# aynik/carta1

Hardware: AMD Instinct MI355X
Metric: atrac1_stereo_frames_per_s_encode (higher is better)
Workload: dtype f32+f64

## Files before the change

### carta1_amd/csrc/c1_k_analysis.hip

```cpp
#include "c1_device.h"

namespace {

struct alignas(16) LongLds {
  float d1[46];
  float d2[46];
  uint32_t late[4][64];
  uint32_t sfw[64];
  double win[32];
  alignas(16) float hbuf[296];
  alignas(4) uint8_t sfi[64];
  union alignas(16) {
    struct { alignas(16) double w1[698]; } q1;
    struct { alignas(16) double w2[454]; } q2;
    struct {
      union alignas(16) {
        struct { alignas(16) float in0[256]; alignas(16) float in1[256]; alignas(16) float in2[512]; } i;
        struct { alignas(16) float coef[512]; } c;
      } a;
      union alignas(16) { float band[512]; } zz;
    } m;
    struct { alignas(16) float skip_[896]; float2 z[320]; } zp;
  } u;
};

struct alignas(16) MixedLds {
  double d1[46];
  double d2[46];
  alignas(16) float band[512];
  alignas(16) float hbuf[296];
  alignas(4) uint8_t sfi[64];
  alignas(16) float ovl[96];
  union alignas(16) {
    struct { alignas(16) double w1[698]; } q1;
    struct { alignas(16) double w2[454]; } q2;
    struct {
      union alignas(16) {
        struct { alignas(16) float in[1120]; } g;
        struct { alignas(16) float coef[512]; } c;
      } a;
      union alignas(16) { float2 z[320]; } zz;
    } m;
  } u;
};

template <bool ALL_LONG>
__global__ __launch_bounds__(C1_WAVE, ALL_LONG ? 4 : 3) void k_analysis_fast(C1EncodeLaunch L) {
  using Lds = typename std::conditional<ALL_LONG, LongLds, MixedLds>::type;
  __shared__ Lds S;
  float *band_;
  if constexpr (ALL_LONG) band_ = S.u.m.zz.band; else band_ = S.band;
  const C1DevEncOpts *O = L.opts;
  const int lane0 = threadIdx.x;
  int lane = lane0;
  const bool listed = L.unit_list != nullptr;
  const int64_t n_items = listed ? (int64_t)*L.unit_count : (int64_t)gridDim.x;
  R4Geometry G4 = r4_geometry(lane0);
  const SfLong SFL = sf_long_geometry(lane0);
  if constexpr (ALL_LONG) {
#pragma unroll
    for (int j = 0; j < 4; j++) {
      S.late[j][lane0] = r4_late_word(G4, j);
      G4.cx[j] = G4.cy[j] = G4.post_tab[j] = 0;
    }
    S.sfw[lane0] = (uint32_t)SFL.src | ((uint32_t)SFL.b << 13) | (SFL.wide ? 1u << 19 : 0u) | (SFL.store ? 1u << 20 : 0u);
    if (lane0 < 32) S.win[lane0] = C1_TABLES(L.tables)->window[lane0];
  }
  const SfLong SFM = sf_geometry(lane0, O->modes[0], O->modes[1], O->modes[2]);
  const MixGeometry GM = mix_geometry(lane0, FrameModes{O->modes[0], O->modes[1], O->modes[2]});
  const TablesRsrc RT = tables_rsrc(L.tables);
  for (int64_t item = blockIdx.x; item < n_items; item += gridDim.x) {
  const int64_t listed_unit = listed ? (int64_t)L.unit_list[item] : 0;
  const int ch = listed ? (int)(listed_unit % L.channels) : (int)(blockIdx.x % L.channels);
  const int64_t f0 = listed ? listed_unit / L.channels : (int64_t)(blockIdx.x / L.channels) * L.run_frames;
  const int64_t run_frames = listed ? (L.list_runs ? (f0 / L.run_frames + 1) * L.run_frames - f0 : 1) : L.run_frames;
  const float *__restrict__ pcm = L.pcm[ch];
  lane = lane0;

  for (int i = lane; i < 46; i += 64) { S.d1[i] = 0.0; S.d2[i] = 0.0; }
  for (int i = lane; i < 296; i += 64) S.hbuf[i] = 0.0f;
  if (lane < 12) S.sfi[52 + lane] = 0;
  if constexpr (!ALL_LONG) {
    for (int i = lane; i < 96; i += 64) S.ovl[i] = 0.0f;
  }
  float ov0 = 0.0f, ov1 = 0.0f, ov2 = 0.0f;
  wave_fence();

  const int64_t f_end = (f0 + run_frames < L.frames) ? f0 + run_frames : L.frames;
  constexpr int kWarm = 1;
  int64_t f_first = f0 - kWarm;
  if (f_first < -(int64_t)L.halo_frames) f_first = -(int64_t)L.halo_frames;
  if (f_first > f0) f_first = f0;
  typedef float v4f __attribute__((ext_vector_type(4)));
  v4f pre_a, pre_b;
  auto deliver = [&]() {
    asm volatile("" : "+v"(pre_a), "+v"(pre_b));
  };
  {
    const v4f *p4 = reinterpret_cast<const v4f *>(pcm + f_first * 512);
    pre_a = p4[lane0]; pre_b = p4[64 + lane0];
    deliver();
  }
  for (int64_t f = f_first; f < f_end; ++f) {
    const bool emit = (f >= f0);
    TablesPtr T = tables_for_this_frame(L.tables);
    lane = lane_for_this_frame(lane0);

    {
      const v4f a = pre_a, b = pre_b;
      {
        const v4f *p4 = reinterpret_cast<const v4f *>(pcm + ((f + 1 < f_end) ? f + 1 : f) * 512);
        pre_a = p4[lane]; pre_b = p4[64 + lane];
      }
      double *w1 = S.u.q1.w1;
      if (lane < 46) w1[pidx<3>(lane)] = S.d1[lane];
      const int e0 = 46 + 4 * lane;
      *reinterpret_cast<double2 *>(&w1[pidx<3>(e0)]) = make_double2((double)a.x, (double)a.y);
      *reinterpret_cast<double2 *>(&w1[pidx<3>(e0 + 2)]) = make_double2((double)a.z, (double)a.w);
      *reinterpret_cast<double2 *>(&w1[pidx<3>(e0 + 256)]) = make_double2((double)b.x, (double)b.y);
      *reinterpret_cast<double2 *>(&w1[pidx<3>(e0 + 258)]) = make_double2((double)b.z, (double)b.w);
    }
    wave_fence();
    {
      double ev[4], od[4];
      if constexpr (ALL_LONG) __builtin_amdgcn_s_setprio(3);
      if (own_block()) qmf_analysis_core<4, 3>(S.u.q1.w1, lane, T, ev, od); else { for (int d = 0; d < 4; d++) { ev[d] = S.u.q1.w1[lane + d]; od[d] = 1.0; } }
      double *w2 = S.u.q2.w2;
      if (lane < 46) { w2[pidx<2>(lane)] = S.d2[lane]; S.d1[lane] = S.u.q1.w1[pidx<3>(512 + lane)]; }
      float lo[4];
#pragma unroll
      for (int d = 0; d < 4; d++) {
        lo[d] = f32(ev[d] + od[d]);
        S.hbuf[39 + 4 * lane + d] = f32(ev[d] - od[d]);
      }
      *reinterpret_cast<double2 *>(&w2[pidx<2>(46 + 4 * lane)]) = make_double2((double)lo[0], (double)lo[1]);
      *reinterpret_cast<double2 *>(&w2[pidx<2>(48 + 4 * lane)]) = make_double2((double)lo[2], (double)lo[3]);
    }
    wave_fence();
    R4Early EARLY;
    if constexpr (ALL_LONG) EARLY = r4_early(G4, RT);
    {
      double ev[2], od[2];
      if (own_block()) qmf_analysis_core<2, 2>(S.u.q2.w2, lane, T, ev, od); else { for (int d = 0; d < 2; d++) { ev[d] = S.u.q2.w2[lane + d]; od[d] = 1.0; } }
      if constexpr (ALL_LONG) __builtin_amdgcn_s_setprio(1);
      *reinterpret_cast<float2 *>(&band_[2 * lane]) = make_float2(f32(ev[0] + od[0]), f32(ev[1] + od[1]));
      *reinterpret_cast<float2 *>(&band_[128 + 2 * lane]) = make_float2(f32(ev[0] - od[0]), f32(ev[1] - od[1]));
      *reinterpret_cast<float4 *>(&band_[256 + 4 * lane]) = *reinterpret_cast<const float4 *>(&S.hbuf[4 * lane]);
      if (lane < 46) S.d2[lane] = S.u.q2.w2[pidx<2>(256 + lane)];
    }
    wave_fence();
    {
      float keep = 0.0f;
      if (lane < 39) keep = S.hbuf[256 + lane];
      wave_fence();
      if (lane < 39) S.hbuf[lane] = keep;
    }
    deliver();
    if (emit && L.bands) {
      float4 *dst = reinterpret_cast<float4 *>(L.bands + ((f * L.channels + ch) << 9));
      const float4 *src = reinterpret_cast<const float4 *>(band_);
      dst[lane] = src[lane];
      dst[64 + lane] = src[64 + lane];
    }

    if constexpr (ALL_LONG) {
      float *in0 = S.u.m.a.i.in0, *in1 = S.u.m.a.i.in1, *in2 = S.u.m.a.i.in2;
      float nov0 = 0.0f, nov1 = 0.0f, nov2 = 0.0f;
      if (lane < 32) {
        const double w_lo = S.win[lane], w_hi = S.win[31 - lane];
        const double x0 = band_[96 + lane], x1 = band_[128 + 96 + lane], x2 = band_[256 + 224 + lane];
        nov0 = f32(w_lo * x0); nov1 = f32(w_lo * x1); nov2 = f32(w_lo * x2);
        if (emit) {
          in0[48 + lane] = ov0; in1[48 + lane] = ov1; in2[112 + lane] = ov2;
          in0[80 + 96 + lane] = f32(x0 * w_hi);
          in1[80 + 96 + lane] = f32(x1 * w_hi);
          in2[144 + 224 + lane] = f32(x2 * w_hi);
        }
      }
      ov0 = nov0; ov1 = nov1; ov2 = nov2;
      if (!emit) { wave_fence(); continue; }
      {
        const float4 zero4 = make_float4(0.0f, 0.0f, 0.0f, 0.0f);
        if (lane < 48) {
          float *inb = lane < 24 ? in0 : in1;
          const int q = lane < 24 ? lane : lane - 24;
          *reinterpret_cast<float4 *>(&inb[q < 12 ? 4 * q : 208 + 4 * (q - 12)]) = zero4;
        }
        if (lane < 56) *reinterpret_cast<float4 *>(&in2[lane < 28 ? 4 * lane : 400 + 4 * (lane - 28)]) = zero4;
        if (lane < 48) {
          *reinterpret_cast<float2 *>(&in0[80 + 2 * lane]) = *reinterpret_cast<const float2 *>(&band_[2 * lane]);
          *reinterpret_cast<float2 *>(&in1[80 + 2 * lane]) = *reinterpret_cast<const float2 *>(&band_[128 + 2 * lane]);
        }
        if (lane < 56) *reinterpret_cast<float4 *>(&in2[144 + 4 * lane]) = *reinterpret_cast<const float4 *>(&band_[256 + 4 * lane]);
      }
      wave_fence();
      float *coef = S.u.m.a.c.coef;
      __builtin_amdgcn_s_setprio(0);
      mdct_long_r4(in0, S.u.zp.z, coef, G4, T, RT, EARLY, &S.late[0][0] + lane);
      __builtin_amdgcn_s_setprio(1);
      wave_fence();

      const int64_t unit = f * L.channels + ch;
      {
        const uint32_t sw = S.sfw[lane];
        const float4 *grp = reinterpret_cast<const float4 *>(coef + (sw & 0x1fcu));
        float mx = sf_scan_long_groups(grp[0], grp[1], grp[2]);
        const float other = __int_as_float(__builtin_amdgcn_update_dpp(0, __float_as_int(mx), 0xB1, 0xf, 0xf, false));
        mx = fmaxf(mx, ((sw >> 19) & 1u) ? other : 0.0f);
        const int sfi = scale_factor_index_fast(mx, T->sf_m1, T->sf_m2);
        if ((sw >> 20) & 1u) S.sfi[(sw >> 13) & 63u] = (uint8_t)sfi;
      }
      {
        float4 *dst = reinterpret_cast<float4 *>(L.coefs + (unit << 9));
        const float4 *src = reinterpret_cast<const float4 *>(coef);
        dst[lane] = src[lane];
        dst[64 + lane] = src[64 + lane];
      }
      wave_fence();
      if (lane < 16) reinterpret_cast<uint32_t *>(L.side + unit * kSideBytes)[lane] = reinterpret_cast<const uint32_t *>(S.sfi)[lane];
      if ((L.list_runs || L.list_zero_eps) && lane == 16) *reinterpret_cast<float4 *>(L.eps + unit * kEpsFloats) = make_float4(0.0f, 0.0f, 0.0f, 0.0f);
      wave_fence();
    } else {
      const FrameModes M{O->modes[0], O->modes[1], O->modes[2]};
      float *coef = S.u.m.a.c.coef;
      if (emit) {
        mix_stage(band_, S.ovl, S.u.m.a.g.in, M, lane, RT);
        wave_fence();
        mdct_mixed_r4(S.u.m.a.g.in, S.u.m.zz.z, coef, GM, M.m0 == 0 || M.m1 == 0 || M.m2 == 0, M.m2 == 0, T, RT);
      }
      for (int i = lane; i < 96; i += 64) {
        const int b = i >> 5, k = i & 31;
        const int Sb = b == 2 ? 256 : 128, off = b == 0 ? 0 : (b == 1 ? 128 : 256);
        S.ovl[i] = f32(T->window[k] * (double)band_[off + Sb - 32 + k]);
      }
      wave_fence();
      if (!emit) continue;

      const int64_t unit = f * L.channels + ch;
      {
        float4 *dst = reinterpret_cast<float4 *>(L.coefs + (unit << 9));
        const float4 *src = reinterpret_cast<const float4 *>(coef);
        dst[lane] = src[lane];
        dst[64 + lane] = src[64 + lane];
      }
      sf_long(coef, S.sfi, SFM, T);
      if (lane >= 60 && lane < 63) reinterpret_cast<uint32_t *>(S.sfi)[13 + (lane - 60)] = lane == 60 ? (uint32_t)((M.m0 & 3) | ((M.m1 & 3) << 2) | ((M.m2 & 3) << 4)) : 0u;
      wave_fence();
      if (lane < 16) reinterpret_cast<uint32_t *>(L.side + unit * kSideBytes)[lane] = reinterpret_cast<const uint32_t *>(S.sfi)[lane];
      if ((L.list_runs || L.list_zero_eps) && lane == 16) *reinterpret_cast<float4 *>(L.eps + unit * kEpsFloats) = make_float4(0.0f, 0.0f, 0.0f, 0.0f);
      wave_fence();
    }
  }
  wave_fence();
  }
}

}

void c1k_launch_analysis(const C1EncodeLaunch &L0, bool detect, hipStream_t stream) {
  static const int slots = c1k_wave_slots(k_analysis_fast<false>);
  C1EncodeLaunch L = L0;
  L.run_frames = c1k_pick_run(L.frames, L.channels, slots);
  const int64_t runs = (L.frames + L.run_frames - 1) / L.run_frames;
  const int64_t blocks = L.unit_list ? std::min<int64_t>(L.frames * L.channels, 256 * 12) : runs * L.channels;
  const dim3 grid((unsigned)blocks), block(C1_WAVE);
  (void)detect;
  hipLaunchKernelGGL((k_analysis_fast<false>), grid, block, 0, stream, L);
}
void c1k_launch_analysis_long(const C1EncodeLaunch &L0, hipStream_t stream) {
  static const int slots = c1k_wave_slots(k_analysis_fast<true>);
  C1EncodeLaunch L = L0;
  L.run_frames = c1k_pick_run(L.frames, L.channels, slots);
  const int64_t runs = (L.frames + L.run_frames - 1) / L.run_frames;
  const int64_t blocks = L.unit_list ? std::min<int64_t>(L.frames * L.channels, 256 * 16) : runs * L.channels;
  hipLaunchKernelGGL((k_analysis_fast<true>), dim3((unsigned)blocks), dim3(C1_WAVE), 0, stream, L);
}
static_assert(sizeof(LongLds) <= 10240, "all-long analysis: 16 waves per CU (4 per SIMD, 128 registers) need <= 10 KiB of LDS per wave");
```

Measured before the change: 197.6 million.

## Specialise all-long analysis kernel with contiguous LDS QMF windows and cross-item prefetch

```diff
diff --git a/carta1_amd/csrc/c1_k_analysis.hip b/carta1_amd/csrc/c1_k_analysis.hip
--- a/carta1_amd/csrc/c1_k_analysis.hip
+++ b/carta1_amd/csrc/c1_k_analysis.hip
@@ -1,17 +1,18 @@
 #include "c1_device.h"
 
+#include <cstddef>
+
 namespace {
 
 struct alignas(16) LongLds {
-  float d1[46];
-  float d2[46];
   uint32_t late[4][64];
   uint32_t sfw[64];
   double win[32];
-  alignas(16) float hbuf[296];
+  double d2[48];
   alignas(4) uint8_t sfi[64];
+  alignas(16) double h1[60];
   union alignas(16) {
-    struct { alignas(16) double w1[698]; } q1;
+    struct { alignas(16) double w1_body[638]; } q1;
     struct { alignas(16) double w2[454]; } q2;
     struct {
       union alignas(16) {
@@ -22,7 +23,13 @@
     } m;
     struct { alignas(16) float skip_[896]; float2 z[320]; } zp;
   } u;
+  float hi_tail[64];
 };
+constexpr int kLongW1 = offsetof(LongLds, h1), kLongUnion = offsetof(LongLds, u), kLongBand = kLongUnion + 4096;
+static_assert(kLongUnion - kLongW1 == 60 * 8, "w1's head ends where its body starts");
+static_assert(sizeof(LongLds::u) == 6144 && offsetof(LongLds, hi_tail) == kLongBand + 2048, "hi_tail continues band");
+static_assert(kLongW1 % 16 == 0 && kLongUnion % 16 == 0, "16-byte window reads");
+static_assert(sizeof(LongLds) <= 10240, "all-long analysis: 16 waves per CU (4 per SIMD, 128 registers) need <= 10 KiB of LDS per wave");
 
 struct alignas(16) MixedLds {
   double d1[46];
@@ -45,27 +52,15 @@
 };
 
 template <bool ALL_LONG>
-__global__ __launch_bounds__(C1_WAVE, ALL_LONG ? 4 : 3) void k_analysis_fast(C1EncodeLaunch L) {
-  using Lds = typename std::conditional<ALL_LONG, LongLds, MixedLds>::type;
-  __shared__ Lds S;
-  float *band_;
-  if constexpr (ALL_LONG) band_ = S.u.m.zz.band; else band_ = S.band;
+__global__ __launch_bounds__(C1_WAVE, 3) void k_analysis_fast(C1EncodeLaunch L) {
+  static_assert(!ALL_LONG, "the all-long kernel is the specialisation below");
+  __shared__ MixedLds S;
+  float *band_ = S.band;
   const C1DevEncOpts *O = L.opts;
   const int lane0 = threadIdx.x;
   int lane = lane0;
   const bool listed = L.unit_list != nullptr;
   const int64_t n_items = listed ? (int64_t)*L.unit_count : (int64_t)gridDim.x;
-  R4Geometry G4 = r4_geometry(lane0);
-  const SfLong SFL = sf_long_geometry(lane0);
-  if constexpr (ALL_LONG) {
-#pragma unroll
-    for (int j = 0; j < 4; j++) {
-      S.late[j][lane0] = r4_late_word(G4, j);
-      G4.cx[j] = G4.cy[j] = G4.post_tab[j] = 0;
-    }
-    S.sfw[lane0] = (uint32_t)SFL.src | ((uint32_t)SFL.b << 13) | (SFL.wide ? 1u << 19 : 0u) | (SFL.store ? 1u << 20 : 0u);
-    if (lane0 < 32) S.win[lane0] = C1_TABLES(L.tables)->window[lane0];
-  }
   const SfLong SFM = sf_geometry(lane0, O->modes[0], O->modes[1], O->modes[2]);
   const MixGeometry GM = mix_geometry(lane0, FrameModes{O->modes[0], O->modes[1], O->modes[2]});
   const TablesRsrc RT = tables_rsrc(L.tables);
@@ -80,10 +75,7 @@
   for (int i = lane; i < 46; i += 64) { S.d1[i] = 0.0; S.d2[i] = 0.0; }
   for (int i = lane; i < 296; i += 64) S.hbuf[i] = 0.0f;
   if (lane < 12) S.sfi[52 + lane] = 0;
-  if constexpr (!ALL_LONG) {
-    for (int i = lane; i < 96; i += 64) S.ovl[i] = 0.0f;
-  }
-  float ov0 = 0.0f, ov1 = 0.0f, ov2 = 0.0f;
+  for (int i = lane; i < 96; i += 64) S.ovl[i] = 0.0f;
   wave_fence();
 
   const int64_t f_end = (f0 + run_frames < L.frames) ? f0 + run_frames : L.frames;
@@ -123,7 +115,6 @@
     wave_fence();
     {
       double ev[4], od[4];
-      if constexpr (ALL_LONG) __builtin_amdgcn_s_setprio(3);
       if (own_block()) qmf_analysis_core<4, 3>(S.u.q1.w1, lane, T, ev, od); else { for (int d = 0; d < 4; d++) { ev[d] = S.u.q1.w1[lane + d]; od[d] = 1.0; } }
       double *w2 = S.u.q2.w2;
       if (lane < 46) { w2[pidx<2>(lane)] = S.d2[lane]; S.d1[lane] = S.u.q1.w1[pidx<3>(512 + lane)]; }
@@ -137,12 +128,9 @@
       *reinterpret_cast<double2 *>(&w2[pidx<2>(48 + 4 * lane)]) = make_double2((double)lo[2], (double)lo[3]);
     }
     wave_fence();
-    R4Early EARLY;
-    if constexpr (ALL_LONG) EARLY = r4_early(G4, RT);
     {
       double ev[2], od[2];
       if (own_block()) qmf_analysis_core<2, 2>(S.u.q2.w2, lane, T, ev, od); else { for (int d = 0; d < 2; d++) { ev[d] = S.u.q2.w2[lane + d]; od[d] = 1.0; } }
-      if constexpr (ALL_LONG) __builtin_amdgcn_s_setprio(1);
       *reinterpret_cast<float2 *>(&band_[2 * lane]) = make_float2(f32(ev[0] + od[0]), f32(ev[1] + od[1]));
       *reinterpret_cast<float2 *>(&band_[128 + 2 * lane]) = make_float2(f32(ev[0] - od[0]), f32(ev[1] - od[1]));
       *reinterpret_cast<float4 *>(&band_[256 + 4 * lane]) = *reinterpret_cast<const float4 *>(&S.hbuf[4 * lane]);
@@ -163,64 +151,7 @@
       dst[64 + lane] = src[64 + lane];
     }
 
-    if constexpr (ALL_LONG) {
-      float *in0 = S.u.m.a.i.in0, *in1 = S.u.m.a.i.in1, *in2 = S.u.m.a.i.in2;
-      float nov0 = 0.0f, nov1 = 0.0f, nov2 = 0.0f;
-      if (lane < 32) {
-        const double w_lo = S.win[lane], w_hi = S.win[31 - lane];
-        const double x0 = band_[96 + lane], x1 = band_[128 + 96 + lane], x2 = band_[256 + 224 + lane];
-        nov0 = f32(w_lo * x0); nov1 = f32(w_lo * x1); nov2 = f32(w_lo * x2);
-        if (emit) {
-          in0[48 + lane] = ov0; in1[48 + lane] = ov1; in2[112 + lane] = ov2;
-          in0[80 + 96 + lane] = f32(x0 * w_hi);
-          in1[80 + 96 + lane] = f32(x1 * w_hi);
-          in2[144 + 224 + lane] = f32(x2 * w_hi);
-        }
-      }
-      ov0 = nov0; ov1 = nov1; ov2 = nov2;
-      if (!emit) { wave_fence(); continue; }
-      {
-        const float4 zero4 = make_float4(0.0f, 0.0f, 0.0f, 0.0f);
-        if (lane < 48) {
-          float *inb = lane < 24 ? in0 : in1;
-          const int q = lane < 24 ? lane : lane - 24;
-          *reinterpret_cast<float4 *>(&inb[q < 12 ? 4 * q : 208 + 4 * (q - 12)]) = zero4;
-        }
-        if (lane < 56) *reinterpret_cast<float4 *>(&in2[lane < 28 ? 4 * lane : 400 + 4 * (lane - 28)]) = zero4;
-        if (lane < 48) {
-          *reinterpret_cast<float2 *>(&in0[80 + 2 * lane]) = *reinterpret_cast<const float2 *>(&band_[2 * lane]);
-          *reinterpret_cast<float2 *>(&in1[80 + 2 * lane]) = *reinterpret_cast<const float2 *>(&band_[128 + 2 * lane]);
-        }
-        if (lane < 56) *reinterpret_cast<float4 *>(&in2[144 + 4 * lane]) = *reinterpret_cast<const float4 *>(&band_[256 + 4 * lane]);
-      }
-      wave_fence();
-      float *coef = S.u.m.a.c.coef;
-      __builtin_amdgcn_s_setprio(0);
-      mdct_long_r4(in0, S.u.zp.z, coef, G4, T, RT, EARLY, &S.late[0][0] + lane);
-      __builtin_amdgcn_s_setprio(1);
-      wave_fence();
-
-      const int64_t unit = f * L.channels + ch;
-      {
-        const uint32_t sw = S.sfw[lane];
-        const float4 *grp = reinterpret_cast<const float4 *>(coef + (sw & 0x1fcu));
-        float mx = sf_scan_long_groups(grp[0], grp[1], grp[2]);
-        const float other = __int_as_float(__builtin_amdgcn_update_dpp(0, __float_as_int(mx), 0xB1, 0xf, 0xf, false));
-        mx = fmaxf(mx, ((sw >> 19) & 1u) ? other : 0.0f);
-        const int sfi = scale_factor_index_fast(mx, T->sf_m1, T->sf_m2);
-        if ((sw >> 20) & 1u) S.sfi[(sw >> 13) & 63u] = (uint8_t)sfi;
-      }
-      {
-        float4 *dst = reinterpret_cast<float4 *>(L.coefs + (unit << 9));
-        const float4 *src = reinterpret_cast<const float4 *>(coef);
-        dst[lane] = src[lane];
-        dst[64 + lane] = src[64 + lane];
-      }
-      wave_fence();
-      if (lane < 16) reinterpret_cast<uint32_t *>(L.side + unit * kSideBytes)[lane] = reinterpret_cast<const uint32_t *>(S.sfi)[lane];
-      if ((L.list_runs || L.list_zero_eps) && lane == 16) *reinterpret_cast<float4 *>(L.eps + unit * kEpsFloats) = make_float4(0.0f, 0.0f, 0.0f, 0.0f);
-      wave_fence();
-    } else {
+    {
       const FrameModes M{O->modes[0], O->modes[1], O->modes[2]};
       float *coef = S.u.m.a.c.coef;
       if (emit) {
@@ -252,6 +183,243 @@
     }
   }
   wave_fence();
+  }
+}
+
+template <int D, int S>
+__device__ __forceinline__ void qmf_core_long(const double *w, int lane, TablesPtr T, double (&even)[D], double (&odd)[D]) {
+  static_assert(2 * D == (1 << S), "the lane base is affine only then");
+  const double *base = w + (2 * D + 2) * lane;
+#pragma unroll
+  for (int d = 0; d < D; d++) even[d] = odd[d] = 0.0;
+#pragma unroll
+  for (int u = 22 + D; u >= 0; --u) {
+    constexpr int kTwo = 2;
+    const int q = kTwo + 2 * u;
+    const double2 x = *reinterpret_cast<const double2 *>(base + (q + 2 * (q >> S)));
+#pragma unroll
+    for (int d = 0; d < D; d++) {
+      const int j = d + 23 - u;
+      if (j >= 0 && j < 24) {
+        odd[d] = __builtin_fma(x.x, T->tap_e[23 - j], odd[d]);
+        even[d] = __builtin_fma(x.y, T->tap_e[j], even[d]);
+      }
+    }
+  }
+}
+
+struct LongItem {
+  int ch;
+  int64_t f0, f_first, f_end;
+};
+
+template <>
+__global__ __launch_bounds__(C1_WAVE, 4) void k_analysis_fast<true>(C1EncodeLaunch L) {
+  __shared__ LongLds S;
+  double *const w1 = reinterpret_cast<double *>(reinterpret_cast<char *>(&S) + kLongW1);
+  double *const w2 = S.u.q2.w2;
+  float *const band_ = reinterpret_cast<float *>(reinterpret_cast<char *>(&S) + kLongBand);
+  const int lane0 = threadIdx.x;
+  int lane = lane0;
+  const bool listed = L.unit_list != nullptr;
+  const int64_t n_items = listed ? (int64_t)*L.unit_count : (int64_t)gridDim.x;
+  if ((int64_t)blockIdx.x >= n_items) return;
+  R4Geometry G4 = r4_geometry(lane0);
+  const SfLong SFL = sf_long_geometry(lane0);
+#pragma unroll
+  for (int j = 0; j < 4; j++) {
+    S.late[j][lane0] = r4_late_word(G4, j);
+    G4.cx[j] = G4.cy[j] = G4.post_tab[j] = 0;
+  }
+  S.sfw[lane0] = (uint32_t)SFL.src | ((uint32_t)SFL.b << 13) | (SFL.wide ? 1u << 19 : 0u) | (SFL.store ? 1u << 20 : 0u);
+  if (lane0 < 32) S.win[lane0] = C1_TABLES(L.tables)->window[lane0];
+  if (lane0 < 12) S.sfi[52 + lane0] = 0;
+  const TablesRsrc RT = tables_rsrc(L.tables);
+
+  auto item_of = [&](uint32_t unit) -> LongItem {
+    LongItem I;
+    int64_t run;
+    if (listed) {
+      const uint32_t nch = (uint32_t)L.channels;
+      uint32_t fr;
+      if (nch == 2u) { I.ch = (int)(unit & 1u); fr = unit >> 1; }
+      else if (nch == 1u) { I.ch = 0; fr = unit; }
+      else { I.ch = (int)(unit % nch); fr = unit / nch; }
+      I.f0 = (int64_t)fr;
+      run = L.list_runs ? (int64_t)((uint32_t)L.run_frames - fr % (uint32_t)L.run_frames) : 1;
+    } else {
+      I.ch = (int)(blockIdx.x % L.channels);
+      I.f0 = (int64_t)(blockIdx.x / L.channels) * L.run_frames;
+      run = L.run_frames;
+    }
+    I.f_end = (I.f0 + run < L.frames) ? I.f0 + run : L.frames;
+    constexpr int kWarm = 1;
+    I.f_first = I.f0 - kWarm;
+    if (I.f_first < -(int64_t)L.halo_frames) I.f_first = -(int64_t)L.halo_frames;
+    if (I.f_first > I.f0) I.f_first = I.f0;
+    return I;
+  };
+  typedef const __attribute__((address_space(4))) uint32_t *ListPtr;
+  auto word_at = [&](int64_t i) -> uint32_t { return (listed && i < n_items) ? ((ListPtr)L.unit_list)[i] : 0u; };
+
+  typedef float v4f __attribute__((ext_vector_type(4)));
+  v4f pre_a, pre_b;
+  auto deliver = [&]() {
+    asm volatile("" : "+v"(pre_a), "+v"(pre_b));
+  };
+  int64_t item = blockIdx.x;
+  uint32_t word = word_at(item), word_next = word_at(item + gridDim.x);
+  {
+    const LongItem I = item_of(__builtin_amdgcn_readfirstlane(word));
+    const v4f *p4 = reinterpret_cast<const v4f *>(L.pcm[I.ch] + I.f_first * 512);
+    pre_a = p4[lane0]; pre_b = p4[64 + lane0];
+    deliver();
+  }
+  for (;;) {
+  const int64_t next_item = item + gridDim.x;
+  const bool more = next_item < n_items;
+  const uint32_t word_after = word_at(next_item + gridDim.x);
+  const LongItem I = item_of(__builtin_amdgcn_readfirstlane(word));
+  const int ch = I.ch;
+  const int64_t f0 = I.f0, f_first = I.f_first, f_end = I.f_end;
+  const float *__restrict__ pcm = L.pcm[ch];
+  const float *after = pcm + (f_end - 1) * 512;
+  if (more) {
+    const LongItem N = item_of(__builtin_amdgcn_readfirstlane(word_next));
+    after = L.pcm[N.ch] + N.f_first * 512;
+  }
+  lane = lane0;
+
+  if (f_first == f0) {
+    if (lane < 60) w1[lane] = 0.0;
+    if (lane < 48) S.d2[lane] = 0.0;
+    band_[512 + lane] = 0.0f;
+  }
+  float ov0 = 0.0f, ov1 = 0.0f, ov2 = 0.0f;
+  wave_fence();
+
+  for (int64_t f = f_first; f < f_end; ++f) {
+    const bool emit = (f >= f0);
+    TablesPtr T = tables_for_this_frame(L.tables);
+    lane = lane_for_this_frame(lane0);
+
+    {
+      const v4f a = pre_a, b = pre_b;
+      {
+        const v4f *p4 = reinterpret_cast<const v4f *>((f + 1 < f_end) ? pcm + (f + 1) * 512 : after);
+        pre_a = p4[lane]; pre_b = p4[64 + lane];
+      }
+      double *at = w1 + (60 + 5 * lane - (lane & 1));
+      *reinterpret_cast<double2 *>(at) = make_double2((double)a.x, (double)a.y);
+      *reinterpret_cast<double2 *>(at + 2) = make_double2((double)a.z, (double)a.w);
+      *reinterpret_cast<double2 *>(at + 320) = make_double2((double)b.x, (double)b.y);
+      *reinterpret_cast<double2 *>(at + 322) = make_double2((double)b.z, (double)b.w);
+    }
+    wave_fence();
+    {
+      double ev[4], od[4];
+      __builtin_amdgcn_s_setprio(3);
+      if (own_block()) qmf_core_long<4, 3>(w1, lane, T, ev, od); else { for (int d = 0; d < 4; d++) { ev[d] = w1[lane + d]; od[d] = 1.0; } }
+      if (lane < 48) {
+        const int h1 = lane + 2 * (lane >> 3), h2 = lane + 2 * (lane >> 2);
+        w1[h1] = w1[640 + h1];
+        w2[h2] = S.d2[lane];
+      }
+      float lo[4], hi[4];
+#pragma unroll
+      for (int d = 0; d < 4; d++) {
+        lo[d] = f32(ev[d] + od[d]);
+        hi[d] = f32(ev[d] - od[d]);
+      }
+      const float pushed = band_[512 + lane];
+      if (lane < 39) band_[256 + lane] = pushed;
+      band_[295 + 4 * lane] = hi[0];
+      *reinterpret_cast<float2 *>(&band_[296 + 4 * lane]) = make_float2(hi[1], hi[2]);
+      band_[298 + 4 * lane] = hi[3];
+      *reinterpret_cast<double2 *>(&w2[72 + 6 * lane]) = make_double2((double)lo[0], (double)lo[1]);
+      *reinterpret_cast<double2 *>(&w2[74 + 6 * lane]) = make_double2((double)lo[2], (double)lo[3]);
+    }
+    wave_fence();
+    R4Early EARLY = r4_early(G4, RT);
+    {
+      double ev[2], od[2];
+      if (own_block()) qmf_core_long<2, 2>(w2, lane, T, ev, od); else { for (int d = 0; d < 2; d++) { ev[d] = w2[lane + d]; od[d] = 1.0; } }
+      __builtin_amdgcn_s_setprio(1);
+      *reinterpret_cast<float2 *>(&band_[2 * lane]) = make_float2(f32(ev[0] + od[0]), f32(ev[1] + od[1]));
+      *reinterpret_cast<float2 *>(&band_[128 + 2 * lane]) = make_float2(f32(ev[0] - od[0]), f32(ev[1] - od[1]));
+      if (lane < 48) S.d2[lane] = w2[384 + lane + 2 * (lane >> 2)];
+    }
+    wave_fence();
+    deliver();
+    if (emit && L.bands) {
+      float4 *dst = reinterpret_cast<float4 *>(L.bands + ((f * L.channels + ch) << 9));
+      const float4 *src = reinterpret_cast<const float4 *>(band_);
+      dst[lane] = src[lane];
+      dst[64 + lane] = src[64 + lane];
+    }
+
+    float *in0 = S.u.m.a.i.in0, *in1 = S.u.m.a.i.in1, *in2 = S.u.m.a.i.in2;
+    float nov0 = 0.0f, nov1 = 0.0f, nov2 = 0.0f;
+    if (lane < 32) {
+      const double w_lo = S.win[lane], w_hi = S.win[31 - lane];
+      const double x0 = band_[96 + lane], x1 = band_[128 + 96 + lane], x2 = band_[256 + 224 + lane];
+      nov0 = f32(w_lo * x0); nov1 = f32(w_lo * x1); nov2 = f32(w_lo * x2);
+      if (emit) {
+        in0[48 + lane] = ov0; in1[48 + lane] = ov1; in2[112 + lane] = ov2;
+        in0[80 + 96 + lane] = f32(x0 * w_hi);
+        in1[80 + 96 + lane] = f32(x1 * w_hi);
+        in2[144 + 224 + lane] = f32(x2 * w_hi);
+      }
+    }
+    ov0 = nov0; ov1 = nov1; ov2 = nov2;
+    if (!emit) { wave_fence(); continue; }
+    {
+      const float4 zero4 = make_float4(0.0f, 0.0f, 0.0f, 0.0f);
+      if (lane < 48) {
+        float *inb = lane < 24 ? in0 : in1;
+        const int q = lane < 24 ? lane : lane - 24;
+        *reinterpret_cast<float4 *>(&inb[q < 12 ? 4 * q : 208 + 4 * (q - 12)]) = zero4;
+      }
+      if (lane < 56) *reinterpret_cast<float4 *>(&in2[lane < 28 ? 4 * lane : 400 + 4 * (lane - 28)]) = zero4;
+      if (lane < 48) {
+        *reinterpret_cast<float2 *>(&in0[80 + 2 * lane]) = *reinterpret_cast<const float2 *>(&band_[2 * lane]);
+        *reinterpret_cast<float2 *>(&in1[80 + 2 * lane]) = *reinterpret_cast<const float2 *>(&band_[128 + 2 * lane]);
+      }
+      if (lane < 56) *reinterpret_cast<float4 *>(&in2[144 + 4 * lane]) = *reinterpret_cast<const float4 *>(&band_[256 + 4 * lane]);
+    }
+    wave_fence();
+    float *coef = S.u.m.a.c.coef;
+    __builtin_amdgcn_s_setprio(0);
+    mdct_long_r4(in0, S.u.zp.z, coef, G4, T, RT, EARLY, &S.late[0][0] + lane);
+    __builtin_amdgcn_s_setprio(1);
+    wave_fence();
+
+    const int64_t unit = f * L.channels + ch;
+    {
+      const uint32_t sw = S.sfw[lane];
+      const float4 *grp = reinterpret_cast<const float4 *>(coef + (sw & 0x1fcu));
+      float mx = sf_scan_long_groups(grp[0], grp[1], grp[2]);
+      const float other = __int_as_float(__builtin_amdgcn_update_dpp(0, __float_as_int(mx), 0xB1, 0xf, 0xf, false));
+      mx = fmaxf(mx, ((sw >> 19) & 1u) ? other : 0.0f);
+      const int sfi = scale_factor_index_fast(mx, T->sf_m1, T->sf_m2);
+      if ((sw >> 20) & 1u) S.sfi[(sw >> 13) & 63u] = (uint8_t)sfi;
+    }
+    {
+      float4 *dst = reinterpret_cast<float4 *>(L.coefs + (unit << 9));
+      const float4 *src = reinterpret_cast<const float4 *>(coef);
+      dst[lane] = src[lane];
+      dst[64 + lane] = src[64 + lane];
+    }
+    wave_fence();
+    if (lane < 16) reinterpret_cast<uint32_t *>(L.side + unit * kSideBytes)[lane] = reinterpret_cast<const uint32_t *>(S.sfi)[lane];
+    if ((L.list_runs || L.list_zero_eps) && lane == 16) *reinterpret_cast<float4 *>(L.eps + unit * kEpsFloats) = make_float4(0.0f, 0.0f, 0.0f, 0.0f);
+    wave_fence();
+  }
+  wave_fence();
+  if (!more) break;
+  item = next_item;
+  word = word_next;
+  word_next = word_after;
   }
 }
 
@@ -275,4 +443,3 @@
   const int64_t blocks = L.unit_list ? std::min<int64_t>(L.frames * L.channels, 256 * 16) : runs * L.channels;
   hipLaunchKernelGGL((k_analysis_fast<true>), dim3((unsigned)blocks), dim3(C1_WAVE), 0, stream, L);
 }
-static_assert(sizeof(LongLds) <= 10240, "all-long analysis: 16 waves per CU (4 per SIMD, 128 registers) need <= 10 KiB of LDS per wave");
```

Result: no change. 199.2 million, median of 6 (+0.8%).
